# slinderman/pyglm

Hardware: AMD Instinct MI355X
Metric: Gibbs sweeps/sec (full resample_model) (higher is better)
Workload: dtype f64 (likelihood Gram: exact integer arithmetic on 13 i8 residue planes, CRT back to f64)

## Files before the change

### pyglm_amd/csrc/pgl_common.h

```cpp
#pragma once
#include <hip/hip_runtime.h>
#include <stdint.h>
#include <stddef.h>
#include <atomic>
#include "../../include/pyglm_hip.h"

#define PGL_OK 0
#define PGL_ERR_ARG 1
#define PGL_ERR_HIP 2

void pgl_set_error(const char* fmt, ...);

#ifdef PGL_AB
#include <cstdlib>
inline int pgl_ab_int(const char* name, int dflt) { const char* e = getenv(name); return e ? atoi(e) : dflt; }
#else
constexpr int pgl_ab_int(const char*, int dflt) { return dflt; }
#endif

constexpr int PGL_MAX_DEVICES = 32;
int pgl_device();
int pgl_device_cus(int dev);
struct PglPerDevice {
    std::atomic<uint32_t> mask{0};
    bool done(int dev) const { return (mask.load(std::memory_order_acquire) >> (dev & 31)) & 1u; }
    void mark(int dev) { mask.fetch_or(1u << (dev & 31), std::memory_order_release); }
};
int pgl_set_dynamic_lds(const void* fn, size_t bytes, PglPerDevice& flag);
struct PglPerDeviceSize { std::atomic<size_t> set[PGL_MAX_DEVICES]; };
int pgl_grow_dynamic_lds(const void* fn, size_t bytes, PglPerDeviceSize& have);

#define PGL_CHECK_ARG(cond)                                                              \
    do {                                                                                 \
        if (!(cond)) {                                                                   \
            pgl_set_error("%s:%d: argument check failed: %s", __FILE__, __LINE__, #cond); \
            return PGL_ERR_ARG;                                                          \
        }                                                                                \
    } while (0)

#define PGL_CHECK_LAUNCH()                                                                         \
    do {                                                                                           \
        hipError_t e_ = hipGetLastError();                                                         \
        if (e_ != hipSuccess) {                                                                    \
            pgl_set_error("%s:%d: kernel launch failed: %s", __FILE__, __LINE__, hipGetErrorString(e_)); \
            return PGL_ERR_HIP;                                                                    \
        }                                                                                          \
    } while (0)

typedef double d4_t __attribute__((ext_vector_type(4)));
typedef double d2_t __attribute__((ext_vector_type(2)));

struct PglGemmArgs {
    const double* A; long lda; long strideA;
    const double* B; long ldb; long strideB;
    double* C; long ldc; long strideC;
    const double* W; long ldw;
    int M, N, K;
    int a_cols, b_cols;
    int nbatch;
    int nz_total;
    double alpha, beta;
    int tri;
    const int* batch_k;
    int* sched;
    const int* batch_dim; int dim_off;
    int dim_mode;
    const int* batch_row_off;
    int pipe;
    int ksplit; long ks_rows; double* Cpart; long part_stride_z, part_stride_s;
};
enum PglGemmKind { PGL_GEMM_GRAM2 = 0, PGL_GEMM_PLAIN = 1, PGL_GEMM_TRI1 = 2, PGL_GEMM_SQUARES = 3 };
int pgl_launch_gemm(PglGemmKind kind, const PglGemmArgs& a, hipStream_t st);
int pgl_gram_split(const double* X, long ldx, int x_cols, const double* W, long ldw, int Tp, int D, int nz, double* J, long ldj, long strideJ, int accumulate,
                   long ks_rows, double* part, long part_stride_z, hipStream_t st);
bool pgl_update_supported(const PglGemmArgs& a);
int pgl_launch_update(const PglGemmArgs& a, hipStream_t st);
int pgl_launch_update_rows(const PglGemmArgs& a, int row0, int nrows, hipStream_t st);
int* pgl_sched_slot(hipStream_t st);

int pgl_k_philox_words(uint64_t, uint32_t, uint32_t, uint64_t, uint64_t, uint32_t*, size_t, hipStream_t);
int pgl_k_pg_draw(const double*, const double*, double*, size_t, uint64_t, uint64_t, uint64_t, hipStream_t);
int pgl_k_row_stats(const int* a, const double* W, double* out, int N, int B, int nloc, int n0, hipStream_t st);
int pgl_k_colsum_partials(const double* part, int nblk, int ncol, double* out, int accumulate, hipStream_t st);
int pgl_k_summary_state(const int* a, const double* Wt, long ldw, const double* bias, double* edge, double* wmean, double* wM2, double* bmean,
                        double* bM2, int N, int B, int nloc, int k, hipStream_t st);
int pgl_k_summary_colsum(const double* V, long ldv, int T, int nloc, double* part, double* out, int accumulate, hipStream_t st);
int pgl_k_scaled_gram(const double*, long, const double*, double*, long, long, int, int, hipStream_t);
int pgl_k_basis_conv(const double*, long, const double*, double*, long, double*, long, int, int, int, int, int, hipStream_t);
int pgl_k_transpose(const double*, long, double*, long, int, int, hipStream_t);
int pgl_k_assemble_post(double*, long, long, const double*, const double*, long, const double*, const double*, const int*, const double*,
                        const double*, int, int, int, hipStream_t);
size_t pgl_k_i8_plane_bytes(int, int);
size_t pgl_k_i8_residue_bytes(int);
int pgl_k_i8_max_planes(void);
int pgl_k_i8_padded_rows(int);
int pgl_k_i8_min_planes(int);
int pgl_k_i8_nu(int, int);
double pgl_k_i8_norm_limit(int, int);
int pgl_k_i8_colstats(const double*, long, const double*, long, int, int, int, double*, double*, hipStream_t);
int pgl_k_i8_scales(const double*, const double*, long, int, int, double*, hipStream_t);
int pgl_k_i8_colmax(const double*, long, int, int, double*, hipStream_t);
int pgl_k_i8_scales_bound(const double*, long, const double*, const double*, int, int, int, int, double*, hipStream_t);
int pgl_k_i8_colstats_scales(const double*, long, const double*, long, int, int, int, int, double*, double*, hipStream_t);
int pgl_k_i8_planes(const double*, long, int transposed, const double*, long, const double*, int8_t*, int, int, int, int, long t_base, hipStream_t);
int pgl_k_i8_gram(const int8_t*, long, int, const int8_t*, int8_t*, int8_t*, int, int, int, int, int, hipStream_t);
long pgl_k_i8_kp(int);
int pgl_k_i8_crt(const int8_t*, const int8_t*, const double*, const double*, double*, long, long, int, int, int, int, hipStream_t);
int pgl_k_flip_apply(const pgl_flip_t&, int, int, int, hipStream_t);
int pgl_k_flip_apply_pair(const pgl_flip_t&, int phase, int window, int* ws, hipStream_t);
int pgl_k_flip_permute(const pgl_flip_t&, const double*, long, long, hipStream_t);
int pgl_k_flip_decide(const pgl_flip_t&, int, hipStream_t);
int pgl_k_flip_pivot_list(const pgl_flip_t&, int*, long, int*, hipStream_t);
int pgl_k_flip_pivot_chunk(const pgl_flip_t&, const int*, long, const int*, int, int, hipStream_t);
int pgl_k_flip_kmax(void);
int pgl_k_flip_window_blocks(int);
int pgl_k_chol_index(const pgl_chol_t&, hipStream_t);
bool pgl_k_small_fits(int N, int B);
int pgl_k_small_max_rows(void);
int pgl_k_small_tail(const double* J, long ldj, long strideJ, int nb, int N, int B, const int* perm, const double* u, const double* rho, const double* c0,
                     int* a, const int* skip, const double* z, long ldz, double* W, double* b, int* status, double* logodds, hipStream_t st);
int pgl_k_chol_sample(const pgl_chol_t&, int, hipStream_t);
```

### pyglm_amd/csrc/pgl_flips.hip

```cpp
#include "pgl_common.h"

namespace {

constexpr int KMAX = 512;
constexpr int KWIN = 320;

struct FlipArgs {
    double* M; long ldj; long strideM;
    int N, B, R;
    const int* perm;
    const double* u;
    const double* rho;
    const double* c0;
    int* a;
    const int* skip;
    int* d_idx;
    double* d_sign;
    int* d_cnt;
    int* batch_k;
    double* G;
    double* Lws;
    double* Ut; double* Wt; long ldu;
    int* status;
    int permuted;
// ... 416 lines not shown
        for (int qi = wave; qi < GT && q0 + qi < kp; qi += 4) {
            const int gq = s_idx[qi];
            Ut[(long)(q0 + qi) * g.ldu + c] = (gq >= 0 && c < Md) ? M[(long)gq * g.ldj + c] : 0.0;
        }
        return;
    }
    const int gq = s_idx[lane];
    for (int ci = wave; ci < GT; ci += 4) {
        const int cc = c0 + ci;
        tile[ci][lane] = (gq >= 0 && cc < Md) ? tab_get(M, g.ldj, gq, cc) : 0.0;
    }
    __syncthreads();
    if (c >= g.ldu) return;
    for (int qi = wave; qi < GT && q0 + qi < kp; qi += 4) Ut[(long)(q0 + qi) * g.ldu + c] = tile[lane][qi];
}

__global__ __launch_bounds__(256) void fixup_kernel(FlipArgs g) {
    const int n = blockIdx.z;
    const int k = g.d_cnt[n];
    const int q0 = blockIdx.y * GT, c0 = blockIdx.x * GT;
    if (k <= 0 || q0 >= k) return;
    const int Md = g.N * g.B + 2;
    const int lane = threadIdx.x & 63, wave = threadIdx.x >> 6;
    double* M = g.M + (long)n * g.strideM;
    const int* idx = g.d_idx + (long)n * KMAX;
    const double* sgn = g.d_sign + (long)n * KMAX;
    const double* Wt = g.Wt + (long)n * KMAX * g.ldu;
    const double* Gn = g.G + (long)n * KMAX * KMAX;
    __shared__ int s_idx[GT];
    __shared__ double s_sg[GT];
    __shared__ int s_piv[GT];
    __shared__ int s_min;
    __shared__ double tile[GT][GT + 1];
    if (threadIdx.x < GT) {
        const bool ok = q0 + threadIdx.x < k;
        s_idx[threadIdx.x] = ok ? idx[q0 + threadIdx.x] : -1;
        s_sg[threadIdx.x] = ok ? sgn[q0 + threadIdx.x] : 0.0;
        s_piv[threadIdx.x] = -1;
    }
    __syncthreads();
    for (int q = threadIdx.x; q < k; q += 256) {
        const int cc = idx[q] - c0;
        if (cc >= 0 && cc < GT) s_piv[cc] = q;
    }
    if (threadIdx.x == 0) {
        int mn = 0x7fffffff;
        for (int i = 0; i < GT; ++i) if (s_idx[i] >= 0 && s_idx[i] < mn) mn = s_idx[i];
        s_min = mn;
    }
    __syncthreads();
    const int c = c0 + lane;
    if (c0 + GT - 1 <= s_min) {
        if (c >= Md) return;
        const int r = s_piv[lane];
        const double sr = r >= 0 ? sgn[r] : 0.0;
        for (int qi = wave; qi < GT; qi += 4) {
            const int gq = s_idx[qi];
            if (gq < 0) break;
            const double v = r < 0 ? s_sg[qi] * Wt[(long)(q0 + qi) * g.ldu + c] : -s_sg[qi] * Gn[(q0 + qi) * KMAX + r] * sr;
            M[(long)gq * g.ldj + c] = v;
        }
        return;
    }
    for (int qi = wave; qi < GT; qi += 4)
        tile[qi][lane] = (s_idx[qi] >= 0 && c < Md) ? s_sg[qi] * Wt[(long)(q0 + qi) * g.ldu + c] : 0.0;
    __syncthreads();
    const int gq = s_idx[lane];
    if (gq < 0) return;
    for (int ci = wave; ci < GT; ci += 4) {
        const int cc = c0 + ci;
        if (cc >= Md) break;
        const int r = s_piv[ci];
        double v;
        if (r < 0) v = tile[lane][ci];
        else { if (gq < cc) continue; v = -s_sg[lane] * Gn[(q0 + lane) * KMAX + r] * sgn[r]; }
        if (gq >= cc) M[(long)gq * g.ldj + cc] = v; else M[(long)cc * g.ldj + gq] = v;
    }
}

__global__ __launch_bounds__(256) void patch_pivot_cols_kernel(FlipArgs g) {
    const int n = blockIdx.y;
    const int k = g.d_cnt[n];
    if (k <= 0) return;
    const int kp = (k + 15) & ~15;
    const int* idx = g.d_idx + (long)n * KMAX;
    const double* sgn = g.d_sign + (long)n * KMAX;
    const double* Gn = g.G + (long)n * KMAX * KMAX;
    double* Wt = g.Wt + (long)n * KMAX * g.ldu;
    double* Ut = g.Ut + (long)n * KMAX * g.ldu;
    for (int e = blockIdx.x * 256 + threadIdx.x; e < kp * k; e += gridDim.x * 256) {
        const int t = e / k, q = e - t * k;
        const double sq = sgn[q];
        Wt[(long)t * g.ldu + idx[q]] = (t == q ? 1.0 : 0.0) - sq * Gn[(long)t * KMAX + q];
        if (t == q) Ut[(long)t * g.ldu + idx[q]] -= sq;
    }
}
__global__ __launch_bounds__(256) void diag_fix_kernel(FlipArgs g) {
    const int n = blockIdx.y, q = blockIdx.x * 256 + threadIdx.x;
    if (q >= g.d_cnt[n]) return;
    const int i = g.d_idx[(long)n * KMAX + q];
    g.M[(long)n * g.strideM + (long)i * g.ldj + i] -= 2.0 * g.d_sign[(long)n * KMAX + q];
}

template <int BT>
__global__ __launch_bounds__(256) void permute_tableau_kernel(FlipArgs g, const double* __restrict__ Jsrc, long lds_, long strideJ) {
    const int n = blockIdx.z, N = g.N, B = BT ? BT : g.B, D = N * B;
    const int* __restrict__ perm = g.perm + (long)n * N;
    const double* __restrict__ J = Jsrc + (long)n * strideJ;
    double* __restrict__ M = g.M + (long)n * g.strideM;
    const int pi = blockIdx.y;
    if (pi < N) {
        const int mi = perm[pi], ncol = (pi + 1) * B;
        for (int c = threadIdx.x; c < ncol; c += 256) {
            const int pj = c / B, y = c - pj * B, mj = perm[pj];
            double v[BT ? BT : 32];
            if (mi > mj) {
#pragma unroll
                for (int x = 0; x < B; ++x) v[x] = J[(long)(mi * B + x) * lds_ + mj * B + y];
            } else if (mi < mj) {
                const double* __restrict__ src = J + (long)(mj * B + y) * lds_ + mi * B;
#pragma unroll
                for (int x = 0; x < B; ++x) v[x] = src[x];
            } else {
#pragma unroll
                for (int x = 0; x < B; ++x) v[x] = tab_get(J, lds_, mi * B + x, mi * B + y);
            }
#pragma unroll
            for (int x = 0; x < B; ++x) M[(long)(pi * B + x) * g.ldj + c] = v[x];
        }
    } else {
        const int row = D + (pi - N);
        for (int c = threadIdx.x; c <= row; c += 256) {
            const int sc = c < D ? perm[c / B] * B + c % B : c;
            M[(long)row * g.ldj + c] = J[(long)row * lds_ + sc];
        }
    }
}

__global__ __launch_bounds__(256) void pivot_list_kernel(FlipArgs g, int* __restrict__ list, long ldl, int* __restrict__ count) {
    const int n = blockIdx.x, tid = threadIdx.x, N = g.N, B = g.B, D = N * B;
    int* L = list + (long)n * ldl;
    if (g.skip && g.skip[n]) { if (tid == 0) count[n] = 0; return; }
    const int* a = g.a + (long)n * N;
    const int* perm = g.perm + (long)n * N;
    __shared__ int s_wave[4];
    __shared__ int s_base;
    if (tid == 0) { s_base = 0; L[0] = D; }
    __syncthreads();
    for (int k0 = 0; k0 < N; k0 += 256) {
        const int k = k0 + tid;
        const int on = k < N ? (a[g.permuted ? perm[k] : k] != 0) : 0;
        const unsigned long long bal = __ballot(on);
        const int lane = tid & 63, wave = tid >> 6;
        const int before = __popcll(bal & ((1ull << lane) - 1ull));
        if (lane == 0) s_wave[wave] = __popcll(bal);
        __syncthreads();
        int off = s_base;
        for (int w = 0; w < wave; ++w) off += s_wave[w];
        if (on) {
            const int p = off + before;
            for (int b = 0; b < B; ++b) L[1 + p * B + b] = k * B + b;
        }
        __syncthreads();
        if (tid == 0) s_base += s_wave[0] + s_wave[1] + s_wave[2] + s_wave[3];
        __syncthreads();
    }
    if (tid == 0) count[n] = 1 + s_base * B;
}

__global__ __launch_bounds__(256) void pivot_chunk_kernel(FlipArgs g, const int* __restrict__ list, long ldl, const int* __restrict__ count, int chunk,
                                                          int per_chunk) {
    const int n = blockIdx.x, tid = threadIdx.x;
    const int begin = chunk * per_chunk;
    int cnt = count[n] - begin;
    cnt = cnt < 0 ? 0 : cnt > per_chunk ? per_chunk : cnt;
    for (int j = tid; j < KMAX; j += 256) {
        g.d_idx[(long)n * KMAX + j] = j < cnt ? list[(long)n * ldl + begin + j] : 0;
        g.d_sign[(long)n * KMAX + j] = 1.0;
    }
    if (tid == 0) g.d_cnt[n] = cnt;
}

}

size_t pgl_k_flip_lds_decide(int B, int R) {
    const int nl = R * B + 1;
    return (2 * (size_t)nl * B + (size_t)B * B + (size_t)R * (B * B + B)) * sizeof(double);
}


int pgl_k_flip_window_blocks(int B) {
    static const int kwin = [] { const int v = pgl_ab_int("PGL_FLIP_WINDOW", KWIN); return v >= 16 && v <= KMAX - 2 ? v : KWIN; }();
    int r = kwin / B;
    while (r > 1 && pgl_k_flip_lds_decide(B, r) > 150 * 1024) --r;
    return r < 1 ? 0 : r;
}

static FlipArgs mk(const pgl_flip_t& s, int R, int c_begin = 0, const int* row_off = nullptr) {
    FlipArgs g{};
    g.M = s.M; g.ldj = s.ldj; g.strideM = s.strideM;
    g.N = s.N; g.B = s.B; g.R = R;
    g.perm = s.perm; g.u = s.u; g.rho = s.rho; g.c0 = s.c0; g.a = s.a; g.skip = s.skip;
    g.d_idx = s.d_idx; g.d_sign = s.d_sign; g.d_cnt = s.d_cnt; g.batch_k = s.batch_k;
    g.G = s.G; g.Lws = s.Lws; g.Ut = s.Ut; g.Wt = s.Wt; g.ldu = s.ldu;
    g.status = s.status; g.permuted = s.visit_order; g.c_begin = c_begin; g.logodds = s.logodds; g.row_off = row_off;
    return g;
}

int pgl_k_flip_apply(const pgl_flip_t& s, int have_G, int max_pivots, int window, hipStream_t st) {
    const int R_ = pgl_k_flip_window_blocks(s.B);
    const int Md_ = s.N * s.B + 2;
    int r0 = 0;
    if (window >= 0 && s.visit_order) {
        if ((long)(window + 1) * R_ >= s.N) return PGL_OK;
        r0 = ((window + 1) * R_ * s.B) & ~1;
    }
    FlipArgs g = mk(s, R_, r0);
    const size_t lds_inv = ((size_t)KMAX + 128 * 129) * sizeof(double);
    static PglPerDevice once;
    if (int rc = pgl_set_dynamic_lds(reinterpret_cast<const void*>(invert_kernel), lds_inv, once)) return rc;
    const int Md = Md_;
    if (!have_G && max_pivots > KB2) {
        if (max_pivots > KMAX) { pgl_set_error("flip_apply: %d pivots per call (max %d)", max_pivots, KMAX); return PGL_ERR_ARG; }
        const int frame = max_pivots > 2 * KB2 ? 4 * KB2 : 2 * KB2;
        const long sq = (long)KMAX * KMAX;
        double* Akk = s.Lws;
        hipLaunchKernelGGL(gather_kk_kernel, dim3(frame * frame / 256, s.nb), dim3(256), 0, st, g, frame);
        PGL_CHECK_LAUNCH();
        auto block_gemm = [&](const double* A, const double* Bm, double* C, double alpha, double beta, int h) {
            PglGemmArgs q{};
            q.A = A; q.lda = KMAX; q.strideA = sq; q.B = Bm; q.ldb = KMAX; q.strideB = sq; q.C = C; q.ldc = KMAX; q.strideC = sq;
            q.M = h; q.N = h; q.K = h; q.a_cols = h; q.b_cols = h; q.nbatch = s.nb; q.alpha = alpha; q.beta = beta; q.tri = 0;
            return pgl_launch_gemm(PGL_GEMM_PLAIN, q, st);
        };
        struct Rec {
            static int inv(const decltype(block_gemm)& gemm, const pgl_flip_t& s, const FlipArgs& g, double* Akk, int o, int n, hipStream_t st) {
                if (n == KB2) {
                    hipLaunchKernelGGL(invert128_kernel, dim3(s.nb), dim3(256), 0, st, g, (const double*)Akk, s.G, o);
                    PGL_CHECK_LAUNCH();
                    return PGL_OK;
                }
                const int h = n / 2;
                int rc = inv(gemm, s, g, Akk, o, h, st);                                               if (rc) return rc;
                double* G_AA = s.G + (long)o * KMAX + o;             double* T = s.G + (long)o * KMAX + o + h;
                double* Tt = s.G + (long)(o + h) * KMAX + o;         double* G_BB = s.G + (long)(o + h) * KMAX + o + h;
                const double* M_AB = Akk + (long)o * KMAX + o + h;   double* S = Akk + (long)(o + h) * KMAX + o + h;
                double* G_BA = Akk + (long)(o + h) * KMAX + o;
                rc = gemm(G_AA, M_AB, T, 1.0, 0.0, h);                                                  if (rc) return rc;
                rc = gemm(M_AB, G_AA, Tt, 1.0, 0.0, h);                                                 if (rc) return rc;
                rc = gemm(M_AB, T, S, -1.0, 1.0, h);                                                    if (rc) return rc;
                rc = inv(gemm, s, g, Akk, o + h, h, st);                                                if (rc) return rc;
                rc = gemm(G_BB, Tt, G_BA, -1.0, 0.0, h);                                                if (rc) return rc;
                rc = gemm(G_BA, Tt, G_AA, -1.0, 1.0, h);                                                if (rc) return rc;
                hipLaunchKernelGGL(offdiag_g_kernel, dim3((h * h + 255) / 256, s.nb), dim3(256), 0, st, g, o, h);
                PGL_CHECK_LAUNCH();
                return PGL_OK;
            }
        };
        int rc = Rec::inv(block_gemm, s, g, Akk, 0, frame, st);
        if (rc) return rc;
        hipLaunchKernelGGL(mask_g_kernel, dim3((KMAX * KMAX + 255) / 256, s.nb), dim3(256), 0, st, g);
        PGL_CHECK_LAUNCH();
    } else if (!have_G) {
        hipLaunchKernelGGL(invert_kernel, dim3(s.nb), dim3(256), lds_inv, st, g);
        PGL_CHECK_LAUNCH();
    }
    hipLaunchKernelGGL(gather_panel_kernel, dim3((unsigned)((s.ldu - r0 + GT - 1) / GT), KMAX / GT, s.nb), dim3(256), 0, st, g);
    PGL_CHECK_LAUNCH();
    const int ncol = (int)s.ldu - r0;
    PglGemmArgs w{};
    w.A = s.G; w.lda = KMAX; w.strideA = (long)KMAX * KMAX;
    w.B = s.Ut + r0; w.ldb = s.ldu; w.strideB = (long)KMAX * s.ldu;
    w.C = s.Wt + r0; w.ldc = s.ldu; w.strideC = (long)KMAX * s.ldu;
    w.M = KMAX; w.N = ncol; w.K = KMAX; w.a_cols = KMAX; w.b_cols = ncol; w.nbatch = s.nb; w.nz_total = 0;
    w.alpha = 1.0; w.beta = 0.0; w.tri = 0; w.batch_k = s.batch_k; w.batch_dim = s.batch_k; w.dim_off = 0; w.dim_mode = 2; w.W = nullptr; w.ldw = 0;
    w.pipe = 1;
    int rc = pgl_launch_gemm(PGL_GEMM_PLAIN, w, st);
    if (rc) return rc;
    static const bool patch_ab = pgl_ab_int("PGL_FLIP_PATCH", 0) != 0;
    const bool patch = r0 == 0 && patch_ab;
    if (patch) {
        hipLaunchKernelGGL(patch_pivot_cols_kernel, dim3(64, s.nb), dim3(256), 0, st, g);
        PGL_CHECK_LAUNCH();
    }
    PglGemmArgs t{};
    t.A = s.Wt + r0; t.lda = s.ldu; t.strideA = (long)KMAX * s.ldu;
    t.B = s.Ut + r0; t.ldb = s.ldu; t.strideB = (long)KMAX * s.ldu;
    t.C = s.M + (long)r0 * s.ldj + r0; t.ldc = s.ldj; t.strideC = s.strideM;
    t.M = Md - r0; t.N = Md - r0; t.K = KMAX; t.a_cols = ncol; t.b_cols = ncol; t.nbatch = s.nb; t.nz_total = 0;
    t.alpha = -1.0; t.beta = 1.0; t.tri = 1; t.batch_k = s.batch_k; t.batch_dim = nullptr; t.dim_off = 0; t.W = nullptr; t.ldw = 0;
    t.pipe = 1;
    rc = pgl_launch_gemm(PGL_GEMM_TRI1, t, st);
    if (rc) return rc;
    if (patch) {
        hipLaunchKernelGGL(diag_fix_kernel, dim3(KMAX / 256, s.nb), dim3(256), 0, st, g);
        PGL_CHECK_LAUNCH();
    } else if (r0 == 0) {
        hipLaunchKernelGGL(fixup_kernel, dim3((Md + GT - 1) / GT, KMAX / GT, s.nb), dim3(256), 0, st, g);
        PGL_CHECK_LAUNCH();
    }
    return PGL_OK;
}

__global__ __launch_bounds__(256) void pair_plan_first_kernel(const int* __restrict__ batch_k, int nb, int room, int* __restrict__ ws) {
    const int n = blockIdx.x * 256 + threadIdx.x;
    if (n >= nb) return;
    const int k1 = batch_k[n];
    const bool paired = k1 + room <= KMAX;
    ws[n] = paired ? k1 : 0;
    ws[nb + n] = paired ? 0 : k1;
    ws[2 * nb + n] = paired ? k1 : 0;
}
__global__ __launch_bounds__(256) void pair_plan_second_kernel(const int* __restrict__ batch_k, int nb, int* __restrict__ ws) {
    const int n = blockIdx.x * 256 + threadIdx.x;
    if (n < nb) ws[3 * nb + n] = ws[n] + batch_k[n];
}

int pgl_k_flip_apply_pair(const pgl_flip_t& s, int phase, int window, int* ws, hipStream_t st) {
    const int R_ = pgl_k_flip_window_blocks(s.B);
    const int Md = s.N * s.B + 2;
    if (!s.visit_order || (long)(window + 1) * R_ >= s.N) return PGL_OK;
    const int r0 = ((window + 1) * R_ * s.B) & ~1;
    FlipArgs g = mk(s, R_, r0, phase ? ws : nullptr);
    hipLaunchKernelGGL(gather_panel_kernel, dim3((unsigned)((s.ldu - r0 + GT - 1) / GT), KMAX / GT, s.nb), dim3(256), 0, st, g);
    PGL_CHECK_LAUNCH();
    const int ncol = (int)s.ldu - r0;
    PglGemmArgs w{};
    w.A = s.G; w.lda = KMAX; w.strideA = (long)KMAX * KMAX;
    w.B = s.Ut + r0; w.ldb = s.ldu; w.strideB = (long)KMAX * s.ldu;
    w.C = s.Wt + r0; w.ldc = s.ldu; w.strideC = (long)KMAX * s.ldu;
    w.M = KMAX; w.N = ncol; w.K = KMAX; w.a_cols = KMAX; w.b_cols = ncol; w.nbatch = s.nb;
    w.alpha = 1.0; w.beta = 0.0; w.tri = 0; w.batch_k = s.batch_k; w.batch_dim = s.batch_k; w.dim_off = 0; w.dim_mode = 2;
    w.batch_row_off = phase ? ws : nullptr;
    w.pipe = 1;
    if (int rc = pgl_launch_gemm(PGL_GEMM_PLAIN, w, st)) return rc;
    PglGemmArgs t{};
    t.A = s.Wt + r0; t.lda = s.ldu; t.strideA = (long)KMAX * s.ldu;
    t.B = s.Ut + r0; t.ldb = s.ldu; t.strideB = (long)KMAX * s.ldu;
    t.C = s.M + (long)r0 * s.ldj + r0; t.ldc = s.ldj; t.strideC = s.strideM;
    t.M = Md - r0; t.N = Md - r0; t.K = KMAX; t.a_cols = ncol; t.b_cols = ncol; t.nbatch = s.nb;
    t.alpha = -1.0; t.beta = 1.0; t.tri = 1; t.pipe = 1;
    if (phase == 0) {
        const int room = (R_ * s.B + 15) & ~15;
        hipLaunchKernelGGL(pair_plan_first_kernel, dim3((s.nb + 255) / 256), dim3(256), 0, st, s.batch_k, s.nb, room, ws);
        PGL_CHECK_LAUNCH();
        t.batch_k = ws + s.nb;
        if (int rc = pgl_launch_gemm(PGL_GEMM_TRI1, t, st)) return rc;
        const int nblk1 = min(R_, s.N - (window + 1) * R_);
        PglGemmArgs q = t;
        q.N = (window + 1) * R_ * s.B + nblk1 * s.B - r0; q.tri = 0; q.pipe = 0; q.batch_k = ws + 2 * s.nb;
        return pgl_launch_gemm(PGL_GEMM_PLAIN, q, st);
    }
    hipLaunchKernelGGL(pair_plan_second_kernel, dim3((s.nb + 255) / 256), dim3(256), 0, st, s.batch_k, s.nb, ws);
    PGL_CHECK_LAUNCH();
    t.batch_k = ws + 3 * s.nb;
    return pgl_launch_gemm(PGL_GEMM_TRI1, t, st);
}

int pgl_k_flip_permute(const pgl_flip_t& s, const double* J, long ldjs, long strideJ, hipStream_t st) {
    FlipArgs g = mk(s, 0);
    g.permuted = 1;
    const dim3 grid(1, s.N + 2, s.nb);
#define PGL_PERMUTE(b_) case b_: hipLaunchKernelGGL(permute_tableau_kernel<b_>, grid, dim3(256), 0, st, g, J, ldjs, strideJ); break;
    switch (s.B) {
        PGL_PERMUTE(1) PGL_PERMUTE(2) PGL_PERMUTE(3) PGL_PERMUTE(4) PGL_PERMUTE(5) PGL_PERMUTE(6) PGL_PERMUTE(7) PGL_PERMUTE(8)
        default: hipLaunchKernelGGL(permute_tableau_kernel<0>, grid, dim3(256), 0, st, g, J, ldjs, strideJ); break;
    }
#undef PGL_PERMUTE
    PGL_CHECK_LAUNCH();
    return PGL_OK;
}

int pgl_k_flip_decide(const pgl_flip_t& s, int window, hipStream_t st) {
    const int R = pgl_k_flip_window_blocks(s.B);
    if (R < 1) { pgl_set_error("B=%d exceeds the window capacity %d", s.B, KWIN); return PGL_ERR_ARG; }
    FlipArgs g = mk(s, R);
    const size_t lds = pgl_k_flip_lds_decide(s.B, R);
#define PGL_DECIDE(b_)                                                                                                      \
    case b_: {                                                                                                              \
        static PglPerDeviceSize lds_set_b;                                                                                  \
        if (int rc = pgl_grow_dynamic_lds(reinterpret_cast<const void*>(decide_kernel<b_>), lds, lds_set_b)) return rc;     \
        hipLaunchKernelGGL(decide_kernel<b_>, dim3(s.nb), dim3(1024), lds, st, g, window);                                  \
    } break;
    switch (s.B <= 8 ? s.B : 0) {
        PGL_DECIDE(0) PGL_DECIDE(1) PGL_DECIDE(2) PGL_DECIDE(3) PGL_DECIDE(4) PGL_DECIDE(5) PGL_DECIDE(6) PGL_DECIDE(7) PGL_DECIDE(8)
        default: break;
    }
#undef PGL_DECIDE
    PGL_CHECK_LAUNCH();
    return PGL_OK;
}

int pgl_k_flip_pivot_list(const pgl_flip_t& s, int* list, long ldl, int* count, hipStream_t st) {
    FlipArgs g = mk(s, 0);
    hipLaunchKernelGGL(pivot_list_kernel, dim3(s.nb), dim3(256), 0, st, g, list, ldl, count);
    PGL_CHECK_LAUNCH();
    return PGL_OK;
}

int pgl_k_flip_pivot_chunk(const pgl_flip_t& s, const int* list, long ldl, const int* count, int chunk, int per_chunk, hipStream_t st) {
    if (per_chunk < 1 || per_chunk > KMAX) { pgl_set_error("pivot chunk of %d rows (max %d)", per_chunk, KMAX); return PGL_ERR_ARG; }
    FlipArgs g = mk(s, 0);
    hipLaunchKernelGGL(pivot_chunk_kernel, dim3(s.nb), dim3(256), 0, st, g, list, ldl, count, chunk, per_chunk);
    PGL_CHECK_LAUNCH();
    return PGL_OK;
}

int pgl_k_flip_kmax(void) { return KMAX; }
```

### pyglm_amd/csrc/pgl_sweep.hip

```cpp
#include "pgl_common.h"
#include "pgl_obs.h"
#include <cmath>
#include <tuple>
#include <vector>

namespace {

__global__ __launch_bounds__(256) void pack_weights_kernel(const int* __restrict__ a, const double* __restrict__ W, const double* __restrict__ b,
                                                           double* __restrict__ Wt, double* __restrict__ bias, int N, int B, int nloc, int Dp, int ldn) {
    const long e = (long)blockIdx.x * 256 + threadIdx.x;
    if (e < nloc) bias[e] = b[e];
    if (e >= (long)Dp * ldn) return;
    const int d = (int)(e / ldn), n = (int)(e % ldn), D = N * B;
    double v = 0.0;
    if (d < D && n < nloc && a[(long)n * N + d / B]) v = W[(long)n * D + d];
    Wt[e] = v;
}

__global__ __launch_bounds__(256) void deterministic_rows_kernel(const double* __restrict__ rho, int* __restrict__ a, int* __restrict__ skip, int N) {
    const int n = blockIdx.x;
    __shared__ int s_any;
    if (threadIdx.x == 0) s_any = 0;
    __syncthreads();
    int bad = 0;
// ... 65 lines not shown
    bool any_i8 = false;
    for (int i = 0; i < s->ndatasets; ++i) {
        const pgl_dataset_t& d = s->datasets[i];
        PGL_CHECK_ARG(d.T > 0 && d.Tp >= d.T && d.Tp % 16 == 0 && d.X && d.Xt && d.OK);
        PGL_CHECK_ARG(!d.int8 || (d.sA && (d.PA || s->i8_PAs) && (d.planes > 0 || s->planes > 0)));
        any_i8 = any_i8 || d.int8;
    }
    PGL_CHECK_ARG(!any_i8 || (s->i8_PB && s->i8_R && s->i8_stat && s->i8_group >= 1 && s->i8_group <= PGL_I8_MAX_GROUP && s->obs != 2));
    return PGL_OK;
}

int sliced_sum(PglGemmKind kind, PglGemmArgs q, long S, double* scratch, double* out, int accumulate, hipStream_t st) {
    const int chunk = (int)(q.K / 16 / S) * 16, rem = q.K - (int)S * chunk;
    q.strideA = (long)chunk * q.lda; q.strideB = (long)chunk * q.ldb; q.C = scratch; q.K = chunk; q.nbatch = (int)S;
    RC(pgl_launch_gemm(kind, q, st));
    if (rem > 0) {
        q.A += (long)S * chunk * q.lda; q.B += (long)S * chunk * q.ldb; q.K = rem; q.nbatch = 1; q.beta = 1.0;
        RC(pgl_launch_gemm(kind, q, st));
    }
    hipLaunchKernelGGL(sum_slices_kernel, dim3((unsigned)((q.strideC + 255) / 256)), dim3(256), 0, st, scratch, q.strideC, (int)S, out, accumulate,
                       (int)q.ldc, q.N);
    PGL_CHECK_LAUNCH();
    return PGL_OK;
}

int gram_batch(const pgl_sweep_t& s, int s0, int nbb, Clock& clk, hipStream_t st) {
    const long D = (long)s.N * s.B;
    const int Dp = r_up(D + 1, 16), ldn = r_up(s.nloc, 2), ldj = r_up(D + 2, 16);
    const long strideJ = (long)ldj * ldj;
    const int kmax = pgl_k_flip_kmax();
    if (s.obs == 2) {
        auto m = clk.tic(ST_GSCALE, 8.0 * nbb * D * (D + 1) / 2);
        RC(pgl_k_scaled_gram(s.G0, ldj, s.inv_eta + s0, s.Jbuf, ldj, strideJ, (int)D, nbb, st));
        clk.toc(m);
        return PGL_OK;
    }
    for (int i = 0; i < s.ndatasets; ++i) {
        const pgl_dataset_t& d = s.datasets[i];
        if (!d.int8) {
            auto m = clk.tic(ST_GRAM, (double)nbb * d.T * D * (D + 1));
            long S = d.Tp / 256;
            if (S > (long)kmax * kmax / ((long)ldj * ldj)) S = (long)kmax * kmax / ((long)ldj * ldj);
            if (S > 64) S = 64;
            if (D <= 512 && S >= 2) {
                const long ks = r_up((d.Tp + S - 1) / S, 16);
                RC(pgl_gram_split(d.X, Dp, Dp, d.OK + s0, 2 * ldn, d.Tp, (int)D, nbb, s.Jbuf, ldj, strideJ, i > 0, ks, s.G, (long)kmax * kmax, st));
            } else RC(pgl_weighted_gram(d.X, Dp, Dp, d.OK + s0, 2 * ldn, d.Tp, (int)D, nbb, s.Jbuf, ldj, strideJ, i > 0, st));
            clk.toc(m);
            continue;
        }
        const int G = s.i8_group, np = d.planes > 0 ? d.planes : s.planes;
        double* sB = s.i8_stat + 2L * G * D;
        const bool batch_norms = d.xmax && s.i8_norm && s0 % 2 == 0;
        const long part = (long)r_up(s.nb, 2) * Dp;
        double* ssb = s.i8_norm;
        double* ommax = s.i8_norm + part;
        if (batch_norms) {
            auto m = clk.tic(ST_STATS, 8.0 * d.T * D);
            RC(pgl_k_i8_colmax(d.OK + s0, 2 * ldn, d.T, nbb, ommax + s0, st));
            const int Mp = r_up(nbb, 2);
            const size_t r_bytes = (size_t)(G < nbb ? G : nbb) * np * pgl_k_i8_padded_rows((int)D) * pgl_k_i8_padded_rows((int)D);
            long S = 64;
            if (S > d.Tp / 256) S = d.Tp / 256;
            if (S > (long)(r_bytes / sizeof(double)) / part) S = (long)(r_bytes / sizeof(double)) / part;
            PglGemmArgs q{};
            q.A = d.OK + s0; q.lda = 2 * ldn; q.a_cols = Mp;
            q.B = d.X; q.ldb = Dp; q.b_cols = Dp;
            q.M = Mp; q.N = (int)D; q.K = d.Tp; q.alpha = 1.0; q.beta = 0.0; q.tri = 0; q.ldc = Dp;
            if (S >= 2) {
                q.strideC = part;
                RC(sliced_sum(PGL_GEMM_SQUARES, q, S, reinterpret_cast<double*>(s.i8_R), ssb, 0, st));
            } else {
                q.C = ssb; q.nbatch = 1;
                RC(pgl_launch_gemm(PGL_GEMM_SQUARES, q, st));
            }
            clk.toc(m);
        }
        for (int g0 = 0; g0 < nbb; g0 += G) {
            const int gz = G < nbb - g0 ? G : nbb - g0;
            const double* om = d.OK + s0 + g0;
            auto m = clk.tic(ST_STATS, batch_norms ? 0.0 : 8.0 * d.T * D);
            if (batch_norms) {
                RC(pgl_k_i8_scales_bound(ssb + (long)g0 * Dp, Dp, ommax + s0 + g0, d.xmax, (int)D, gz, d.T, np, sB, st));
            } else {
                for (int c0 = 0; c0 < gz; c0 += 8) {
                    const int cz = 8 < gz - c0 ? 8 : gz - c0;
                    RC(pgl_k_i8_colstats_scales(d.X, Dp, om + c0, 2 * ldn, d.T, (int)D, cz, np, reinterpret_cast<double*>(s.i8_R), sB + (long)c0 * D, st));
                }
            }
            clk.toc(m);
            const int slice = s.i8_slice > 0 && s.i8_slice < d.T ? s.i8_slice : d.T;
            for (int t0 = 0; t0 < d.T; t0 += slice) {
                const int ts = slice < d.T - t0 ? slice : d.T - t0;
                m = clk.tic(ST_PLANES, (double)np * (gz + (d.PA ? 0 : 1)) * ts * D);
                if (!d.PA) RC(pgl_k_i8_planes(d.Xt + t0, d.Tp, 1, nullptr, 0, d.sA, static_cast<int8_t*>(s.i8_PAs), ts, (int)D, 1, np, t0, st));
                RC(pgl_k_i8_planes(d.Xt + t0, d.Tp, 1, om + (long)t0 * 2 * ldn, 2 * ldn, sB, static_cast<int8_t*>(s.i8_PB), ts, (int)D, gz, np, t0, st));
                clk.toc(m);
                m = clk.tic(ST_I8, (double)gz * ts * D * (D + 1));
                if (d.PA) RC(pgl_k_i8_gram(static_cast<const int8_t*>(d.PA), pgl_k_i8_kp(d.T), t0 / 64, static_cast<const int8_t*>(s.i8_PB),
                                           static_cast<int8_t*>(s.i8_R), static_cast<int8_t*>(s.i8_Rx), ts, (int)D, gz, np, t0 > 0, st));
                else RC(pgl_k_i8_gram(static_cast<const int8_t*>(s.i8_PAs), 0, 0, static_cast<const int8_t*>(s.i8_PB), static_cast<int8_t*>(s.i8_R),
                                      static_cast<int8_t*>(s.i8_Rx), ts, (int)D, gz, np, t0 > 0, st));
                clk.toc(m);
            }
            m = clk.tic(ST_CRT, (double)np * gz * D * (D + 1) / 2);
            RC(pgl_k_i8_crt(static_cast<const int8_t*>(s.i8_R), static_cast<const int8_t*>(s.i8_Rx), d.sA, sB, s.Jbuf + (long)g0 * strideJ, ldj, strideJ, (int)D, gz, np, i > 0, st));
            clk.toc(m);
        }
    }
    return PGL_OK;
}

}

extern "C" {

const char* pgl_stage_name(int i) { return (i >= 0 && i < PGL_NSTAGES) ? STAGE_NAMES[i] : nullptr; }

int pgl_sweep_dims(int N, int B, int nloc, int* Dp, int* ldn, int* ldj) {
    PGL_CHECK_ARG(N > 0 && B > 0 && nloc > 0);
    const long D = (long)N * B;
    if (Dp) *Dp = r_up(D + 1, 16);
    if (ldn) *ldn = r_up(nloc, 2);
    if (ldj) *ldj = r_up(D + 2, 16);
    return PGL_OK;
}

int pgl_stage_times_collect(pgl_stage_times_t* t) {
    PGL_CHECK_ARG(t != nullptr);
    Pending* p = static_cast<Pending*>(t->pending);
    if (!p) return PGL_OK;
    int rc = PGL_OK;
    for (auto& e : p->ev) {
        float ms = 0.f;
        const hipEvent_t e0 = std::get<1>(e), e1 = std::get<2>(e);
        if (hipEventSynchronize(e1) != hipSuccess || hipEventElapsedTime(&ms, e0, e1) != hipSuccess) { pgl_set_error("stage timing: event query failed"); rc = PGL_ERR_HIP; }
        else { const int s = std::get<0>(e); t->ms[s] += ms; t->calls[s] += 1; t->work[s] += std::get<3>(e); }
        (void)hipEventDestroy(e0);
        (void)hipEventDestroy(e1);
    }
    delete p;
    t->pending = nullptr;
    return rc;
}

int pgl_sweep(const pgl_sweep_t* s, uint64_t seed, uint64_t sweep, void* hip_stream) {
    hipStream_t st = reinterpret_cast<hipStream_t>(hip_stream);
    RC(check_gram_args(s));
    PGL_CHECK_ARG(s->B <= 32 && s->n0 >= 0 && (s->obs_param != nullptr || s->obs != 1 || s->xi > 0) && (s->obs_param != nullptr || s->obs != 3 || s->xi >= 0));
    PGL_CHECK_ARG(s->a && s->W && s->b && s->rho && s->Jw && s->hw && s->Jb && s->hb && s->c0 && s->perm && s->u && s->z && s->ll && s->status);
    PGL_CHECK_ARG(s->Wt && s->bias && s->border && s->skip && s->Mtab && s->Ac && s->hc && s->Tinv && s->Lws && s->Ut && s->Wt_ws);
    PGL_CHECK_ARG(s->d_idx && s->d_sign && s->d_cnt && s->batch_k && s->act && s->na && (s->label == nullptr || s->c0_dense != nullptr));
    PGL_CHECK_ARG(s->nrun >= 0 && s->nfirst >= 0 && s->nfirst % 2 == 0 && s->nfirst + s->nrun <= s->nloc && (s->nrun > 0 || s->nfirst == 0));
    for (int i = 0; i < s->ndatasets; ++i) {
        const pgl_dataset_t& d = s->datasets[i];
        PGL_CHECK_ARG(d.Y && d.Psi && d.llpart && (s->obs != 4 || d.hooks));
    }
    const int N = s->N, B = s->B, nloc = s->nloc;
    const int nrun = s->nrun > 0 ? s->nrun : nloc;
    const int nf = s->nfirst;
    const int nb = s->nb < nrun ? s->nb : nrun;
    const long D = (long)N * B;
    const int Dp = r_up(D + 1, 16), ldn = r_up(nloc, 2), ldj = r_up(D + 2, 16);
    const long strideJ = (long)ldj * ldj;
    const int R = pgl_k_flip_window_blocks(B);
    const int kmax = pgl_k_flip_kmax();
    if (R < 1) { pgl_set_error("B=%d too large for the proposal window", B); return PGL_ERR_ARG; }
    Clock clk{s->times, st};

    {
        auto m = clk.tic(ST_PACK);
        const long tot = (long)Dp * ldn;
        hipLaunchKernelGGL(pack_weights_kernel, dim3((unsigned)((tot + 255) / 256)), dim3(256), 0, st, s->a, s->W, s->b, s->Wt, s->bias, N, B, nloc, Dp, ldn);
        PGL_CHECK_LAUNCH();
        clk.toc(m);
    }
    for (int i = 0; i < s->ndatasets; ++i) {
        const pgl_dataset_t& d = s->datasets[i];
        auto m = clk.tic(ST_ACT, 2.0 * d.T * D * nrun);
        {
            PglGemmArgs q{};
            q.A = d.Xt; q.lda = d.Tp; q.a_cols = d.Tp;
            q.B = s->Wt + nf; q.ldb = ldn; q.b_cols = ldn - nf;
            q.C = d.Psi + nf; q.ldc = ldn;
            q.M = d.T; q.N = nrun; q.K = Dp; q.nbatch = 1; q.alpha = 1.0; q.beta = 0.0; q.tri = 0;
            RC(pgl_launch_gemm(PGL_GEMM_PLAIN, q, st));
        }
        clk.toc(m);
        m = clk.tic(ST_PG, (double)d.T * nrun);
        {
            PgLlArgs q{};
            q.Psi = d.Psi + nf; q.ldpsi = ldn; q.bias = s->bias + nf; q.Y = d.Y + nf; q.ldy = ldn; q.llpart = d.llpart; q.T = d.T; q.nloc = nrun;
            q.obs = s->obs; q.xi = s->xi; q.param = s->obs_param ? s->obs_param + nf : nullptr;
            q.hooks = s->obs == 4 ? d.hooks + nf : nullptr; q.ldh = ldn; q.inv_eta = s->obs == 2 ? s->inv_eta + nf : nullptr;
            q.Omega = d.OK + nf; q.ldo = 2 * ldn; q.Kappa = d.OK + ldn + nf; q.ldk = 2 * ldn;
            q.seed = seed; q.sweep = sweep; q.neuron0 = (uint64_t)(s->n0 + nf); q.elem0 = d.elem0;
            RC(pgl_k_pg_loglik(q, s->ll + nf, i > 0, st));
        }
        clk.toc(m);
        if (d.omega_override) {
            if (hipMemcpy2DAsync(d.OK, (size_t)2 * ldn * sizeof(double), d.omega_override, (size_t)nloc * sizeof(double), (size_t)nloc * sizeof(double),
                                 (size_t)d.T, hipMemcpyDeviceToDevice, st) != hipSuccess) { pgl_set_error("omega override copy failed"); return PGL_ERR_HIP; }
        }
    }
    for (int i = 0; i < s->ndatasets; ++i) {
        const pgl_dataset_t& d = s->datasets[i];
        auto m = clk.tic(ST_BORDER, 4.0 * d.T * (D + 1) * nrun);
        const int npieces = nrun < nloc ? 2 : 1;
        const int Mp = nrun < nloc ? r_up(nrun, 2) : 2 * ldn;
        long S = 64;
        if (S > d.Tp / 256) S = d.Tp / 256;
        double* scratch = s->Jbuf;
        long cap_any = (long)ldj * ldj / (4L * Dp), scratch_doubles = (long)nb * strideJ;
        if (cap_any < S && (long)kmax * kmax / (4L * Dp) > cap_any) {
            scratch = s->G;
            cap_any = (long)kmax * kmax / (4L * Dp);
            scratch_doubles = (long)nb * kmax * kmax;
        }
        if (S > cap_any) S = cap_any;
        if (S >= 2) {
            long cols_fit = scratch_doubles / (S * Dp) / 2 * 2;
            const bool whole = npieces == 1 && cols_fit >= 2L * ldn;
            const int cols = nrun < nloc ? r_up(nrun, 2) : ldn;
            const int ngroups_cols = whole ? 2 * ldn : (int)(cols_fit < cols ? cols_fit : cols);
            for (int piece = 0; piece < (whole ? 1 : 2); ++piece) {
                const int first = whole ? 0 : nf, count = whole ? 2 * ldn : cols;
                for (int c0 = 0; c0 < count; c0 += ngroups_cols) {
                    const int mcols = ngroups_cols < count - c0 ? ngroups_cols : count - c0;
                    PglGemmArgs a{};
                    a.A = d.OK + (long)piece * ldn + first + c0; a.lda = 2 * ldn; a.a_cols = mcols;
                    a.B = d.X; a.ldb = Dp; a.b_cols = Dp;
                    a.ldc = Dp; a.strideC = (long)mcols * Dp;
                    a.M = mcols; a.N = (int)D + 1; a.K = d.Tp; a.alpha = 1.0; a.beta = 0.0; a.tri = 0;
                    RC(sliced_sum(PGL_GEMM_PLAIN, a, S, scratch, s->border + ((long)piece * ldn + first + c0) * Dp, i > 0, st));
                }
            }
        } else {
            for (int piece = 0; piece < npieces; ++piece) {
                const double* Ap = d.OK + (long)piece * ldn + nf;
                const long crow = ((long)piece * ldn + nf) * Dp;
                RC(pgl_contract_tn(Ap, 2 * ldn, Mp, d.X, Dp, Dp, s->border + crow, Dp, Mp, (int)D + 1, d.Tp, 1.0, i > 0 ? 1.0 : 0.0, st));
            }
        }
        clk.toc(m);
    }
    hipLaunchKernelGGL(deterministic_rows_kernel, dim3(nloc), dim3(256), 0, st, s->rho, s->a, s->skip, N);
    PGL_CHECK_LAUNCH();
    if (hipMemsetAsync(s->status, 0, (size_t)nloc * sizeof(int), st) != hipSuccess) { pgl_set_error("memset failed"); return PGL_ERR_HIP; }
    if (s->logodds) {
        hipLaunchKernelGGL(fill_kernel, dim3((unsigned)(((long)nloc * N + 255) / 256)), dim3(256), 0, st, s->logodds, (long)nloc * N, (double)NAN);
        PGL_CHECK_LAUNCH();
    }
    const double* c0 = s->c0;
    if (s->label) {
        hipLaunchKernelGGL(gather_table_kernel, dim3((unsigned)(((long)nloc * N + 255) / 256)), dim3(256), 0, st, s->c0, s->label, s->c0_dense, (long)nloc * N);
        PGL_CHECK_LAUNCH();
        c0 = s->c0_dense;
    }

    for (int s0 = nf; s0 < nf + nrun; s0 += nb) {
        const int nbb = nb < nf + nrun - s0 ? nb : nf + nrun - s0;
        RC(gram_batch(*s, s0, nbb, clk, st));
        {
            auto m = clk.tic(ST_ASM);
            const double* jw = s->label ? s->Jw : s->Jw + (long)s0 * N * B * B;
            const double* hw = s->label ? s->hw : s->hw + (long)s0 * N * B;
            const int* lab = s->label ? s->label + (long)s0 * N : nullptr;
            RC(pgl_k_assemble_post(s->Jbuf, ldj, strideJ, s->border + (long)s0 * Dp, s->border + (long)(ldn + s0) * Dp, Dp, jw, hw, lab, s->Jb + s0, s->hb + s0,
                                   nbb, N, B, st));
            clk.toc(m);
        }
        if (s->visit_order && pgl_k_small_fits(N, B)) {
            auto ms = clk.tic(ST_FLIPS);
            RC(pgl_k_small_tail(s->Jbuf, ldj, strideJ, nbb, N, B, s->perm + (long)s0 * N, s->u + (long)s0 * N, s->rho + (long)s0 * N, c0 + (long)s0 * N,
                                s->a + (long)s0 * N, s->skip + s0, s->z + (long)s0 * (D + 1), D + 1, s->W + (long)s0 * D, s->b + s0, s->status + s0,
                                s->logodds ? s->logodds + (long)s0 * N : nullptr, st));
            clk.toc(ms);
            continue;
        }
        auto mf = clk.tic(ST_FLIPS);
        if (!s->all_deterministic) {
            pgl_flip_t fs{};
            fs.M = s->Mtab; fs.ldj = ldj; fs.strideM = strideJ; fs.nb = nbb; fs.N = N; fs.B = B;
            fs.perm = s->perm + (long)s0 * N; fs.u = s->u + (long)s0 * N; fs.rho = s->rho + (long)s0 * N; fs.c0 = c0 + (long)s0 * N;
            fs.a = s->a + (long)s0 * N; fs.skip = s->skip + s0;
            fs.d_idx = s->d_idx; fs.d_sign = s->d_sign; fs.d_cnt = s->d_cnt; fs.batch_k = s->batch_k;
            fs.G = s->G; fs.Lws = s->Lws; fs.Ut = s->Ut; fs.Wt = s->Wt_ws; fs.ldu = ldj;
            fs.status = s->status + s0; fs.visit_order = s->visit_order ? 1 : 0; fs.logodds = s->logodds ? s->logodds + (long)s0 * N : nullptr;
            if (s->visit_order) RC(pgl_k_flip_permute(fs, s->Jbuf, ldj, strideJ, st));
            else if (hipMemcpyAsync(s->Mtab, s->Jbuf, (size_t)nbb * strideJ * sizeof(double), hipMemcpyDeviceToDevice, st) != hipSuccess) {
                pgl_set_error("tableau copy failed"); return PGL_ERR_HIP;
            }
            RC(pgl_k_flip_pivot_list(fs, s->act, D + 1, s->na, st));
            const int ck = kmax;
            long rows = s->init_rows_bound > 0 && s->init_rows_bound <= D + 1 ? s->init_rows_bound : D + 1;
            for (int c = 0; (long)c * ck < rows; ++c) {
                const long left = (D + 1) - (long)c * ck;
                auto m = clk.tic(ST_FINIT);
                RC(pgl_k_flip_pivot_chunk(fs, s->act, D + 1, s->na, c, ck, st));
                RC(pgl_k_flip_apply(fs, 0, (int)(left < ck ? left : ck), -1, st));
                clk.toc(m);
            }
            const int nwin = (N + R - 1) / R;
            const bool pair = s->visit_order && !s->flip_single_pass;
            for (int w = 0; w < nwin; ++w) {
                auto m = clk.tic(ST_FDEC);
                RC(pgl_k_flip_decide(fs, w, st));
                clk.toc(m);
                m = clk.tic(ST_FAPP);
                if (!pair || (w % 2 == 0 && w + 1 >= nwin)) RC(pgl_k_flip_apply(fs, 1, 0, w, st));
                else RC(pgl_k_flip_apply_pair(fs, w % 2, w, s->act, st));
                clk.toc(m);
            }
        }
        clk.toc(mf);
        auto mw = clk.tic(ST_W);
        pgl_chol_t cs{};
        cs.J = s->Jbuf; cs.ldj = ldj; cs.strideJ = strideJ; cs.a = s->a + (long)s0 * N;
        cs.act = s->act; cs.ldact = D + 1; cs.na = s->na;
        cs.Ac = s->Ac; cs.ldc = ldj; cs.strideC = strideJ; cs.hc = s->hc; cs.Tinv = s->Tinv;
        cs.z = s->z + (long)s0 * (D + 1); cs.ldz = D + 1; cs.W = s->W + (long)s0 * D; cs.b = s->b + s0;
        cs.nb = nbb; cs.N = N; cs.B = B; cs.status = s->status + s0;
        RC(pgl_k_chol_index(cs, st));
        long na_bound = s->active_rows_bound > 0 && s->active_rows_bound <= D + 1 ? s->active_rows_bound : D + 1;
        RC(pgl_k_chol_sample(cs, (int)na_bound, st));
        clk.toc(mw);
    }
    return PGL_OK;
}

int pgl_sweep_gram(const pgl_sweep_t* s, int first, int count, void* hip_stream) {
    RC(check_gram_args(s));
    PGL_CHECK_ARG(first >= 0 && count > 0 && count <= s->nb && first + count <= s->nloc);
    hipStream_t st = reinterpret_cast<hipStream_t>(hip_stream);
    Clock clk{s->times, st};
    return gram_batch(*s, first, count, clk, st);
}

int pgl_get_state(const pgl_sweep_t* s, int* a_host, double* W_host, double* b_host, double* ll_host, int* status_host, void* hip_stream) {
    hipStream_t st = reinterpret_cast<hipStream_t>(hip_stream);
    PGL_CHECK_ARG(s && s->nloc > 0);
    const long D = (long)s->N * s->B;
    auto cp = [&](void* dst, const void* src, size_t bytes) { return dst == nullptr || hipMemcpyAsync(dst, src, bytes, hipMemcpyDeviceToHost, st) == hipSuccess; };
    bool ok = cp(a_host, s->a, (size_t)s->nloc * s->N * sizeof(int)) && cp(W_host, s->W, (size_t)s->nloc * D * sizeof(double)) &&
              cp(b_host, s->b, (size_t)s->nloc * sizeof(double)) && cp(ll_host, s->ll, (size_t)s->nloc * sizeof(double)) &&
              cp(status_host, s->status, (size_t)s->nloc * sizeof(int));
    if (!ok || hipStreamSynchronize(st) != hipSuccess) { pgl_set_error("pgl_get_state: copy failed: %s", hipGetErrorString(hipGetLastError())); return PGL_ERR_HIP; }
    return PGL_OK;
}

}
```

Baseline: 0.05929.

## Replace paired flip updates with lazy accumulated low-rank updates and per-window refresh

Replaces the two-phase paired window update of the flip tableau with a lazy scheme. Rank updates accumulate per batch up to KMAX rows, and each window's diagonal block and bias rows are refreshed on demand with a new MFMA f64 product kernel. The full trailing triangular update is flushed only when the accumulated height would overflow. This aims to cut the repeated trailing-matrix GEMM work, at the cost of extra small kernels per window and more complex height bookkeeping.

Result: no change. 0.05957, median of 6 (+0.5%).

```diff
diff --git a/pyglm_amd/csrc/pgl_common.h b/pyglm_amd/csrc/pgl_common.h
--- a/pyglm_amd/csrc/pgl_common.h
+++ b/pyglm_amd/csrc/pgl_common.h
@@ -107,7 +107,9 @@
 long pgl_k_i8_kp(int);
 int pgl_k_i8_crt(const int8_t*, const int8_t*, const double*, const double*, double*, long, long, int, int, int, int, hipStream_t);
 int pgl_k_flip_apply(const pgl_flip_t&, int, int, int, hipStream_t);
-int pgl_k_flip_apply_pair(const pgl_flip_t&, int phase, int window, int* ws, hipStream_t);
+int pgl_k_flip_lazy_begin(const pgl_flip_t&, int* ws, hipStream_t);
+int pgl_k_flip_lazy_refresh(const pgl_flip_t&, int window, const int* ws, hipStream_t);
+int pgl_k_flip_lazy_push(const pgl_flip_t&, int window, int* ws, hipStream_t);
 int pgl_k_flip_permute(const pgl_flip_t&, const double*, long, long, hipStream_t);
 int pgl_k_flip_decide(const pgl_flip_t&, int, hipStream_t);
 int pgl_k_flip_pivot_list(const pgl_flip_t&, int*, long, int*, hipStream_t);
diff --git a/pyglm_amd/csrc/pgl_flips.hip b/pyglm_amd/csrc/pgl_flips.hip
--- a/pyglm_amd/csrc/pgl_flips.hip
+++ b/pyglm_amd/csrc/pgl_flips.hip
@@ -742,28 +742,125 @@
     return PGL_OK;
 }
 
-__global__ __launch_bounds__(256) void pair_plan_first_kernel(const int* __restrict__ batch_k, int nb, int room, int* __restrict__ ws) {
+struct LazyArgs {
+    const double* Wt; const double* Ut; long ldu;
+    const int* height;
+    double* C; long strideC, c_ms, c_ns;
+    const int* c_off;
+    int a_col0;
+    int b_col0; const int* b_idx; const int* b_cnt;
+    int M, N, tri;
+};
+
+__global__ __launch_bounds__(256) void lazy_product_kernel(LazyArgs g) {
+    const int batch = blockIdx.z;
+    const int K = g.height[batch];
+    if (K <= 0) return;
+    const int lane = threadIdx.x & 63, wave = threadIdx.x >> 6;
+    const int frow = lane >> 4, fcol = lane & 15;
+    const int m0 = blockIdx.x * 64 + wave * 16, n0 = blockIdx.y * 32;
+    const int Nv = g.b_cnt ? min(g.b_cnt[batch], g.N) : g.N;
+    if (m0 >= g.M || n0 >= Nv || (g.tri && n0 > m0 + 15)) return;
+    const double* __restrict__ Ab = g.Wt + (long)batch * KMAX * g.ldu;
+    const double* __restrict__ Bb = g.Ut + (long)batch * KMAX * g.ldu;
+    double* __restrict__ Cb = g.C + (long)batch * g.strideC + (g.c_off ? (long)g.c_off[batch] * g.c_ns : 0);
+    auto live = [&](int m, int n) { return m < g.M && n < Nv && (!g.tri || m >= n); };
+    d4_t acc[2];
+#pragma unroll
+    for (int j = 0; j < 2; ++j)
+#pragma unroll
+        for (int r = 0; r < 4; ++r) {
+            const int m = m0 + frow + 4 * r, n = n0 + j * 16 + fcol;
+            acc[j][r] = live(m, n) ? Cb[(long)m * g.c_ms + (long)n * g.c_ns] : 0.0;
+        }
+    const int ca = g.a_col0 + min(m0 + fcol, g.M - 1);
+    int cb[2];
+#pragma unroll
+    for (int j = 0; j < 2; ++j) {
+        const int n = min(n0 + j * 16 + fcol, Nv - 1);
+        cb[j] = g.b_idx ? g.b_idx[(long)batch * KMAX + n] : g.b_col0 + n;
+    }
+    const double* ap = Ab + (long)frow * g.ldu + ca;
+    const double* bp0 = Bb + (long)frow * g.ldu + cb[0];
+    const double* bp1 = Bb + (long)frow * g.ldu + cb[1];
+    const long sk = 4 * g.ldu;
+    for (int k0 = 0; k0 < K; k0 += 32) {
+        double a[8], b0[8], b1[8];
+        const int steps = (K - k0) >= 32 ? 8 : 4;
+#pragma unroll
+        for (int s = 0; s < 8; ++s) {
+            const bool on = s < steps;
+            a[s] = on ? -ap[s * sk] : 0.0;
+            b0[s] = on ? bp0[s * sk] : 0.0;
+            b1[s] = on ? bp1[s * sk] : 0.0;
+        }
+#pragma unroll
+        for (int s = 0; s < 8; ++s) {
+            if (s < steps) {
+                acc[0] = __builtin_amdgcn_mfma_f64_16x16x4f64(a[s], b0[s], acc[0], 0, 0, 0);
+                acc[1] = __builtin_amdgcn_mfma_f64_16x16x4f64(a[s], b1[s], acc[1], 0, 0, 0);
+            }
+        }
+        ap += 8 * sk; bp0 += 8 * sk; bp1 += 8 * sk;
+    }
+#pragma unroll
+    for (int j = 0; j < 2; ++j)
+#pragma unroll
+        for (int r = 0; r < 4; ++r) {
+            const int m = m0 + frow + 4 * r, n = n0 + j * 16 + fcol;
+            if (live(m, n)) Cb[(long)m * g.c_ms + (long)n * g.c_ns] = acc[j][r];
+        }
+}
+
+__global__ __launch_bounds__(256) void lazy_plan_kernel(const int* __restrict__ batch_k, int nb, int room, int* __restrict__ ws) {
     const int n = blockIdx.x * 256 + threadIdx.x;
     if (n >= nb) return;
-    const int k1 = batch_k[n];
-    const bool paired = k1 + room <= KMAX;
-    ws[n] = paired ? k1 : 0;
-    ws[nb + n] = paired ? 0 : k1;
-    ws[2 * nb + n] = paired ? k1 : 0;
-}
-__global__ __launch_bounds__(256) void pair_plan_second_kernel(const int* __restrict__ batch_k, int nb, int* __restrict__ ws) {
-    const int n = blockIdx.x * 256 + threadIdx.x;
-    if (n < nb) ws[3 * nb + n] = ws[n] + batch_k[n];
-}
-
-int pgl_k_flip_apply_pair(const pgl_flip_t& s, int phase, int window, int* ws, hipStream_t st) {
+    const int h = ws[n] + batch_k[n];
+    const bool flush = h + room > KMAX;
+    ws[n] = flush ? 0 : h;
+    ws[nb + n] = flush ? h : 0;
+}
+
+static int lazy_product(const pgl_flip_t& s, const LazyArgs& q, int n_launch, hipStream_t st) {
+    hipLaunchKernelGGL(lazy_product_kernel, dim3((unsigned)((q.M + 63) / 64), (unsigned)((n_launch + 31) / 32), s.nb), dim3(256), 0, st, q);
+    PGL_CHECK_LAUNCH();
+    return PGL_OK;
+}
+
+int pgl_k_flip_lazy_begin(const pgl_flip_t& s, int* ws, hipStream_t st) {
+    if (hipMemsetAsync(ws, 0, 2 * (size_t)s.nb * sizeof(int), st) != hipSuccess) { pgl_set_error("memset failed"); return PGL_ERR_HIP; }
+    return PGL_OK;
+}
+
+int pgl_k_flip_lazy_refresh(const pgl_flip_t& s, int window, const int* ws, hipStream_t st) {
     const int R_ = pgl_k_flip_window_blocks(s.B);
-    const int Md = s.N * s.B + 2;
+    const int D = s.N * s.B, c0 = window * R_ * s.B;
+    const int nrow = min(R_, s.N - window * R_) * s.B;
+    if (!s.visit_order || window <= 0 || nrow <= 0) return PGL_OK;
+    LazyArgs q{};
+    q.Wt = s.Wt; q.Ut = s.Ut; q.ldu = s.ldu; q.height = ws;
+    q.strideC = s.strideM; q.c_ms = s.ldj; q.c_ns = 1;
+    q.b_col0 = c0; q.N = nrow;
+    q.C = s.M + (long)c0 * s.ldj + c0; q.a_col0 = c0; q.M = nrow; q.tri = 1;
+    if (int rc = lazy_product(s, q, nrow, st)) return rc;
+    q.C = s.M + (long)D * s.ldj + c0; q.a_col0 = D; q.M = 2; q.tri = 0;
+    return lazy_product(s, q, nrow, st);
+}
+
+int pgl_k_flip_lazy_push(const pgl_flip_t& s, int window, int* ws, hipStream_t st) {
+    const int R_ = pgl_k_flip_window_blocks(s.B);
+    const int D = s.N * s.B, Md = D + 2;
     if (!s.visit_order || (long)(window + 1) * R_ >= s.N) return PGL_OK;
     const int r0 = ((window + 1) * R_ * s.B) & ~1;
-    FlipArgs g = mk(s, R_, r0, phase ? ws : nullptr);
+    const int room = (R_ * s.B + 15) & ~15;
+    FlipArgs g = mk(s, R_, r0, ws);
     hipLaunchKernelGGL(gather_panel_kernel, dim3((unsigned)((s.ldu - r0 + GT - 1) / GT), KMAX / GT, s.nb), dim3(256), 0, st, g);
     PGL_CHECK_LAUNCH();
+    LazyArgs q{};
+    q.Wt = s.Wt; q.Ut = s.Ut; q.ldu = s.ldu; q.height = ws;
+    q.C = s.Ut + r0; q.strideC = (long)KMAX * s.ldu; q.c_ms = 1; q.c_ns = s.ldu; q.c_off = ws;
+    q.a_col0 = r0; q.M = D - r0; q.b_idx = s.d_idx; q.b_cnt = s.d_cnt; q.N = R_ * s.B; q.tri = 0;
+    if (int rc = lazy_product(s, q, R_ * s.B, st)) return rc;
     const int ncol = (int)s.ldu - r0;
     PglGemmArgs w{};
     w.A = s.G; w.lda = KMAX; w.strideA = (long)KMAX * KMAX;
@@ -771,29 +868,17 @@
     w.C = s.Wt + r0; w.ldc = s.ldu; w.strideC = (long)KMAX * s.ldu;
     w.M = KMAX; w.N = ncol; w.K = KMAX; w.a_cols = KMAX; w.b_cols = ncol; w.nbatch = s.nb;
     w.alpha = 1.0; w.beta = 0.0; w.tri = 0; w.batch_k = s.batch_k; w.batch_dim = s.batch_k; w.dim_off = 0; w.dim_mode = 2;
-    w.batch_row_off = phase ? ws : nullptr;
+    w.batch_row_off = ws;
     w.pipe = 1;
     if (int rc = pgl_launch_gemm(PGL_GEMM_PLAIN, w, st)) return rc;
+    hipLaunchKernelGGL(lazy_plan_kernel, dim3((s.nb + 255) / 256), dim3(256), 0, st, s.batch_k, s.nb, room, ws);
+    PGL_CHECK_LAUNCH();
     PglGemmArgs t{};
     t.A = s.Wt + r0; t.lda = s.ldu; t.strideA = (long)KMAX * s.ldu;
     t.B = s.Ut + r0; t.ldb = s.ldu; t.strideB = (long)KMAX * s.ldu;
     t.C = s.M + (long)r0 * s.ldj + r0; t.ldc = s.ldj; t.strideC = s.strideM;
     t.M = Md - r0; t.N = Md - r0; t.K = KMAX; t.a_cols = ncol; t.b_cols = ncol; t.nbatch = s.nb;
-    t.alpha = -1.0; t.beta = 1.0; t.tri = 1; t.pipe = 1;
-    if (phase == 0) {
-        const int room = (R_ * s.B + 15) & ~15;
-        hipLaunchKernelGGL(pair_plan_first_kernel, dim3((s.nb + 255) / 256), dim3(256), 0, st, s.batch_k, s.nb, room, ws);
-        PGL_CHECK_LAUNCH();
-        t.batch_k = ws + s.nb;
-        if (int rc = pgl_launch_gemm(PGL_GEMM_TRI1, t, st)) return rc;
-        const int nblk1 = min(R_, s.N - (window + 1) * R_);
-        PglGemmArgs q = t;
-        q.N = (window + 1) * R_ * s.B + nblk1 * s.B - r0; q.tri = 0; q.pipe = 0; q.batch_k = ws + 2 * s.nb;
-        return pgl_launch_gemm(PGL_GEMM_PLAIN, q, st);
-    }
-    hipLaunchKernelGGL(pair_plan_second_kernel, dim3((s.nb + 255) / 256), dim3(256), 0, st, s.batch_k, s.nb, ws);
-    PGL_CHECK_LAUNCH();
-    t.batch_k = ws + 3 * s.nb;
+    t.alpha = -1.0; t.beta = 1.0; t.tri = 1; t.pipe = 1; t.batch_k = ws + s.nb;
     return pgl_launch_gemm(PGL_GEMM_TRI1, t, st);
 }
 
diff --git a/pyglm_amd/csrc/pgl_sweep.hip b/pyglm_amd/csrc/pgl_sweep.hip
--- a/pyglm_amd/csrc/pgl_sweep.hip
+++ b/pyglm_amd/csrc/pgl_sweep.hip
@@ -391,14 +391,20 @@
                 clk.toc(m);
             }
             const int nwin = (N + R - 1) / R;
-            const bool pair = s->visit_order && !s->flip_single_pass;
+            const bool lazy = s->visit_order && !s->flip_single_pass;
+            if (lazy) RC(pgl_k_flip_lazy_begin(fs, s->act, st));
             for (int w = 0; w < nwin; ++w) {
+                if (lazy && w > 0) {
+                    auto m = clk.tic(ST_FAPP);
+                    RC(pgl_k_flip_lazy_refresh(fs, w, s->act, st));
+                    clk.toc(m);
+                }
                 auto m = clk.tic(ST_FDEC);
                 RC(pgl_k_flip_decide(fs, w, st));
                 clk.toc(m);
                 m = clk.tic(ST_FAPP);
-                if (!pair || (w % 2 == 0 && w + 1 >= nwin)) RC(pgl_k_flip_apply(fs, 1, 0, w, st));
-                else RC(pgl_k_flip_apply_pair(fs, w % 2, w, s->act, st));
+                if (lazy) RC(pgl_k_flip_lazy_push(fs, w, s->act, st));
+                else RC(pgl_k_flip_apply(fs, 1, 0, w, st));
                 clk.toc(m);
             }
         }
```
